# bark-simulator/planner-miqp

Measured on AMD Instinct MI355X. Metric: MIQP solves/sec to 1% gap, 2-agent x 20-step x 32-region, higher is better.
Workload: dtype f64

## Files before the change

### planner_miqp_amd/csrc/as_onchip.hip

```cpp
namespace miqp {

#ifdef MIQP_PROFILE
#define ASP_T(var) const long long var = clock64()
#define ASP_ACC(k, t0, t1) asp_[k] += (unsigned long long)((t1) - (t0))
#else
#define ASP_T(var)
#define ASP_ACC(k, t0, t1)
#endif
constexpr int AS_MAXSTEP = 220;
constexpr double AS_VTOL = 1.0e-8;
constexpr double AS_DEP = 1.0e-8;
constexpr int AS_MT = 64;
constexpr int AS_MSTR = AS_MT * (AS_MT + 1) / 2;

__host__ __device__ constexpr bool as_shape_ok(int C, int N) { return (C == 1 || C == 2) && N >= 1 && N <= 2 * OC_NSL; }

template <int C> __device__ inline int as_col(int pq) { return C == 2 ? ((pq & 3) << 2) | (pq >> 2) : ((pq & 1) << 2) | (pq >> 1); }
template <int C> __device__ inline int as_pcol(int q) { return C == 2 ? ((q & 3) << 2) | (q >> 2) : ((q & 3) << 1) | (q >> 2); }
template <int C> struct AsDecode {
  static constexpr bool LANE_BOUNDS = true, ROW_IDENTITY = true, MARKS = true;
  static __device__ int col(int l) { return as_col<C>(oc_pcol<C, true>(l)); }
};

template <int C, int NSL, int GCAP = miqp::OC_GCAP>
__global__ void __launch_bounds__(64, (GCAP > 128 ? 1 : 2)) as_onchip_kernel(DevBuf B) {
  static_assert(C == 1 || C == 2, "a stage of 16 columns holds the chains of up to two cars");
  constexpr bool CM = true;
  constexpr bool BIG = GCAP > 128;
  constexpr int OC_GCAP = GCAP, OC_GSLOTS = OC_GCAP / 64, OC_GCOEF = oc_gcoef_of(OC_GCAP);
  constexpr int NX = 6 * C, NZ = 8 * C, NCH = 2 * C;
  const Layout& Y = B.Y;
  const int tid = threadIdx.x, lg = tid >> 4, lc = tid & 15;
  const int par = lg >> 1, side = lg & 1;
  const double bsgn = side ? -1.0 : 1.0;
  WAVE_DUMP(BIG ? 1 : 4);
  const int* const clist = BIG && B.cls_take ? B.cls_list + (size_t)(B.cls_take - 1) * B.batch_cap : nullptr;
  const int nbatch = clist ? (B.cls_count[B.cls_take - 1] < B.batch_cap ? B.cls_count[B.cls_take - 1] : B.batch_cap) : (*B.batch_count < B.batch_cap ? *B.batch_count : B.batch_cap);
  const int N = Y.N, NSLOT = Y.NSLOT;
  extern __shared__ double lds[];
  char* const L0 = (char*)lds;
  const OcLds LL = oc_lds_layout(N, Y.fixlen, OC_GCAP, !BIG);
  double* const Z = (double*)(L0 + LL.z);
  double* const scr = (double*)(L0 + LL.u);
  double* const V = (double*)(L0 + LL.u);
  unsigned long long* const bkey = (unsigned long long*)(L0 + LL.r);
  const int SPAN = LL.gmeta - LL.u;
  double* const kref = (double*)(L0 + LL.u + SPAN - N * 32);
  double* const kff = kref - N * 4;
  double* const KS = kff - N * 16;
  const int STG_CAP = (SPAN - N * 192) / 8;
  uint4* const gmeta = (uint4*)(L0 + LL.gmeta);
  double* const gcoef = (double*)(L0 + LL.gcoef);
  double* const grhs = (double*)(L0 + LL.grhs);
  double* const Wd = (double*)(L0 + LL.wd);
  int* const sstart = (int*)(L0 + LL.sstart);
  unsigned short* const cand = (unsigned short*)(L0 + LL.cand);
  signed char* const fix = (signed char*)(L0 + LL.fix);
  __shared__ int sh_node;
  __shared__ unsigned long long sh_stat[32];
  if (tid < 32) sh_stat[tid] = 0ull;
  const unsigned long long lt = (1ull << tid) - 1ull;

  const int chunk = B.as_chunk > 0 ? B.as_chunk : 1;
  int run_next = 0, run_end = 0;
  const int quota = BIG ? 0 : B.as_quota; int handed = 0;
#ifdef MIQP_PROFILE
  const unsigned long long wv_c0 = __builtin_amdgcn_s_memtime(), wv_r0 = __builtin_amdgcn_s_memrealtime();
  unsigned long long wv_first = 0; int wv_nodes = 0;
  if (!BIG && tid == 0) wv_first = atomicMin(&B.prof[120], wv_r0);
#endif
  for (;;) {
    __syncthreads();
    if (run_next >= run_end) {
      if (quota > 0 && handed >= quota) break;
      ++handed;
      if (tid == 0) sh_node = atomicAdd(B.work_counter, chunk);
      __syncthreads();
      run_next = __builtin_amdgcn_readfirstlane(sh_node); run_end = run_next + chunk;
      if (run_next >= nbatch) break;
    }
    const int slot_ = run_next++;
    if (slot_ >= nbatch) { run_next = run_end; continue; }
    const int node = clist ? __builtin_amdgcn_readfirstlane(clist[slot_]) : slot_;
    {
      const int cls = B.batch_large ? (int)B.batch_large[node] : (is_probe_word(B.batch_depth[node]) ? 1 : 0);
      if (cls != (BIG ? 1 : 0)) continue;
    }
    WAVE_DUMP_NODE();
    const int inst = __builtin_amdgcn_readfirstlane(B.batch_inst[node]);
    const double* D = B.inst_d + (size_t)inst * Y.dstride;
    const int* T = B.inst_i + (size_t)inst * Y.istride;
    const double ts = D[Y.d_glob + 7];
    const double aqs = 2.0 * D[Y.d_misc + 0];
    const double iaq = aqs > 0.0 ? 1.0 / aqs : 0.0;
    {
      const signed char* src = B.pool_fix + (size_t)B.batch_node[node] * Y.fixlen;
      for (int k = tid; k < Y.fixlen; k += 64) fix[k] = src[k];
      if (tid < 16) Wd[tid] = tid < NZ ? D[Y.d_wd + oc_lcol<C, CM>(as_pcol<C>(tid))] : 0.0;
      for (int k = tid; k < N * 32; k += 64) bkey[k] = ~0ull;
      for (int k = tid; k <= N + 1; k += 64) sstart[k] = 0;
    }
    __syncthreads();
    const double* Rf = D + Y.d_ref;
    double cutoff = 1e300;
    {
      const double inc0 = fmin(inc_from_key(*(volatile unsigned long long*)&B.inc_key[inst]), B.inc_ext[inst]);
      const double gap_ = is_probe_word(B.batch_depth[node]) ? 0.0 : B.inst_gap[inst];
      if (B.use_cutoff && inc0 < 1e300) cutoff = inc0 - gap_ * (1e-10 + fabs(inc0)) - B.inst_const[inst];
    }

#ifdef MIQP_PROFILE
    unsigned long long asp_[12] = {0, 0, 0, 0, 0, 0, 0, 0, 0, 0, 0, 0};
#endif
    ASP_T(ta0);
#define OC_DECODE_POLICY AsDecode<C>
#include "oc_decode_body.inc"
#undef OC_DECODE_POLICY
    if (overflow) {
      if (B.batch_A) B.batch_A[(size_t)node * 64 + tid] = 0xFFFFu;
      if (tid == 0) {
        if (B.ring_M) B.batch_Mtag[node] = 0ull;
        B.batch_ok[node] = 5; B.pool_big[B.batch_node[node]] |= (BIG ? 2 : 1); if (B.stats) { atomicAdd(&B.stats[3], 1ull); atomicAdd(&B.stats[8 + (ngen >= 512 ? 15 : ngen / 32)], 1ull); }
      }
      continue;
    }
    const int NM = sstart[N + 1];
    OC_WAVE_SYNC();

    ASP_T(ta1); ASP_ACC(0, ta0, ta1);
#ifdef MIQP_PROFILE
    asp_[9] += (unsigned long long)(ocd_t_sparse - ta0); asp_[11] += (unsigned long long)(ta1 - ocd_t_rows);
#endif
    double brhs[NSL];
    unsigned int bact = 0u, binA = 0u, ginA = 0u;
#pragma unroll
    for (int k = 0; k < NSL; ++k) {
      const int i = 2 * k + par;
      brhs[k] = 1e300;
      if (i < N && lc < NZ) {
        const unsigned long long key = bkey[(i * 2 + side) * 16 + lc];
        if (key != ~0ull) { brhs[k] = key2d(key); bact |= 1u << k; }
      }
    }
    OC_WAVE_SYNC();

    const double h1 = ts, h2 = 0.5 * ts * ts, h3 = ts * ts * ts / 6.0;
    const double* const tb = D + Y.d_astab;
    if constexpr (C == 2) {
      for (int k = tid; k < N * 16; k += 64) KS[k] = tb[k];
      for (int k = tid; k < N * 4; k += 64) kref[k] = tb[N * 16 + k];
    } else {
      for (int k = tid; k < N * 8; k += 64) KS[(k >> 3) * 16 + (k & 7)] = tb[k];
      for (int k = tid; k < N * 2; k += 64) kref[(k >> 1) * 4 + (k & 1)] = tb[N * 8 + k];
    }
    OC_WAVE_SYNC();
    typedef double d2_t __attribute__((ext_vector_type(2)));
    auto subst = [&](const bool fromx0, const int itop, const int iend, double* const out) {
      for (int k = tid; k < (N - 1) * 4; k += 64) if ((k >> 2) > itop) kff[k] = fromx0 ? kref[k] : 0.0;
      if (tid < NCH) {
        const int ch = tid;
        double p0 = 0.0, p1 = 0.0, p2 = 0.0;
        int i0 = itop;
        if (itop >= N - 1) { const d2_t a = *(const d2_t*)(V + (N - 1) * 16 + 4 * ch); p0 = a[0]; p1 = a[1]; p2 = V[(N - 1) * 16 + 4 * ch + 2]; i0 = N - 2; }
        if (i0 >= 0) {
          d2_t va = *(const d2_t*)(V + i0 * 16 + 4 * ch), vb = *(const d2_t*)(V + i0 * 16 + 4 * ch + 2);
          d2_t ka = *(const d2_t*)(KS + (i0 * 4 + ch) * 4), kb = *(const d2_t*)(KS + (i0 * 4 + ch) * 4 + 2);
          double kr = fromx0 ? kref[i0 * 4 + ch] : 0.0;
          for (int i = i0; i >= 0; --i) {
            const int j = i > 0 ? i - 1 : 0;
            const d2_t nva = *(const d2_t*)(V + j * 16 + 4 * ch), nvb = *(const d2_t*)(V + j * 16 + 4 * ch + 2);
            const d2_t nka = *(const d2_t*)(KS + (j * 4 + ch) * 4), nkb = *(const d2_t*)(KS + (j * 4 + ch) * 4 + 2);
            const double nkr = fromx0 ? kref[j * 4 + ch] : 0.0;
            const double su = vb[1] + h3 * p0 + h2 * p1 + h1 * p2;
            const double sx0 = va[0] + p0, sx1 = va[1] + h1 * p0 + p1, sx2 = vb[0] + h2 * p0 + h1 * p1 + p2;
            kff[i * 4 + ch] = fma(su, kb[1], kr);
            p0 = sx0 - ka[0] * su; p1 = sx1 - ka[1] * su; p2 = sx2 - kb[0] * su;
            va = nva; vb = nvb; ka = nka; kb = nkb; kr = nkr;
          }
        }
      }
      OC_WAVE_SYNC();
      if (tid < NCH) {
        const int ch = tid;
        double x0 = 0.0, x1 = 0.0, x2 = 0.0;
        if (fromx0) { const int c = ch >> 1, s = ch & 1; x0 = D[Y.d_x0 + 6 * c + 3 * s]; x1 = D[Y.d_x0 + 6 * c + 3 * s + 1]; x2 = D[Y.d_x0 + 6 * c + 3 * s + 2]; }
        const int ie = iend < N - 1 ? iend : N - 2;
        d2_t ka = *(const d2_t*)(KS + ch * 4), kb = *(const d2_t*)(KS + ch * 4 + 2);
        double kf = kff[ch];
        for (int i = 0; i <= ie; ++i) {
          const int j = i < N - 2 ? i + 1 : N - 2;
          const d2_t nka = *(const d2_t*)(KS + (j * 4 + ch) * 4), nkb = *(const d2_t*)(KS + (j * 4 + ch) * 4 + 2);
          const double nkf = kff[j * 4 + ch];
          const double u = -kf - (ka[0] * x0 + ka[1] * x1 + kb[0] * x2);
          d2_t oa, ob; oa[0] = x0; oa[1] = x1; ob[0] = x2; ob[1] = u;
          *(d2_t*)(out + i * 16 + 4 * ch) = oa; *(d2_t*)(out + i * 16 + 4 * ch + 2) = ob;
          const double n0 = x0 + h1 * x1 + h2 * x2 + h3 * u, n1 = x1 + h1 * x2 + h2 * u, n2 = x2 + h1 * u;
// ... 438 lines not shown
```

### planner_miqp_amd/csrc/kernels.hip

```cpp
#include <hip/hip_runtime.h>

#include "host_inst.hpp"

#ifndef MIQP_RHO
#define MIQP_RHO 1.0e5
#endif

#ifndef MIQP_IPM_WPE
#define MIQP_IPM_WPE 3
#endif

#ifdef MIQP_ABLATE
#define MIQP_ABL (B.abl)
#else
#define MIQP_ABL 0
#endif
namespace miqp {

constexpr double RHO_EL = MIQP_RHO;
constexpr double FEAS_TOL = 1.0e-6;
constexpr double QP_TOL = 1.0e-6;
#ifndef MIQP_T0
#define MIQP_T0 1.0e-3
#endif
// ... 114 lines not shown
  double* ring_M; unsigned long long* ring_head; unsigned long long ring_doubles, ring_margin;
  unsigned long long* batch_Mtag;
  unsigned long long* pool_Mtag;
  int width_cap;
  int as_probe_first;
  int as_chunk;
  int* cls_list;
  int* cls_count;
  int cls_take;
  int lns_warm;
  int as_quota;
  int as_split;
  unsigned long long* as_stats;
};

__device__ inline unsigned long long d2key(double v) {
  unsigned long long u = (unsigned long long)__double_as_longlong(v);
  return (u & 0x8000000000000000ull) ? ~u : (u | 0x8000000000000000ull);
}
__device__ inline double key2d(unsigned long long k) {
  unsigned long long u = (k & 0x8000000000000000ull) ? (k & 0x7FFFFFFFFFFFFFFFull) : ~k;
  return __longlong_as_double((long long)u);
}

__device__ inline double inc_from_key(unsigned long long key) {
  if (key >= 0xFFF0000000000000ull) return 1e300;
  return key2d(key & ~0xFFFFFull);
}

template <int CTRL> __device__ inline double dpp_mov(double x) {
  int lo = __double2loint(x), hi = __double2hiint(x);
  lo = __builtin_amdgcn_update_dpp(lo, lo, CTRL, 0xF, 0xF, false);
  hi = __builtin_amdgcn_update_dpp(hi, hi, CTRL, 0xF, 0xF, false);
  return __hiloint2double(hi, lo);
}
__device__ inline void rows16(double x, double& even, double& odd) {
  const unsigned lo = (unsigned)__double2loint(x), hi = (unsigned)__double2hiint(x);
  const auto a = __builtin_amdgcn_permlane16_swap(lo, lo, false, false);
  const auto b = __builtin_amdgcn_permlane16_swap(hi, hi, false, false);
  even = __hiloint2double((int)b[0], (int)a[0]); odd = __hiloint2double((int)b[1], (int)a[1]);
}
__device__ inline void halves32(double x, double& lower, double& upper) {
  const unsigned lo = (unsigned)__double2loint(x), hi = (unsigned)__double2hiint(x);
  const auto a = __builtin_amdgcn_permlane32_swap(lo, lo, false, false);
  const auto b = __builtin_amdgcn_permlane32_swap(hi, hi, false, false);
  lower = __hiloint2double((int)b[0], (int)a[0]); upper = __hiloint2double((int)b[1], (int)a[1]);
}
__device__ inline double sum_xor16(double v) { double a, b; rows16(v, a, b); return a + b; }
__device__ inline double sum_xor32(double v) { double a, b; halves32(v, a, b); return a + b; }
__device__ inline double wave_min(double v) {
  v = fmin(v, dpp_mov<0xB1>(v)); v = fmin(v, dpp_mov<0x4E>(v)); v = fmin(v, dpp_mov<0x141>(v)); v = fmin(v, dpp_mov<0x140>(v));
  double a, b; rows16(v, a, b); v = fmin(a, b); halves32(v, a, b); return fmin(a, b);
}
__device__ inline double wave_max(double v) {
  v = fmax(v, dpp_mov<0xB1>(v)); v = fmax(v, dpp_mov<0x4E>(v)); v = fmax(v, dpp_mov<0x141>(v)); v = fmax(v, dpp_mov<0x140>(v));
  double a, b; rows16(v, a, b); v = fmax(a, b); halves32(v, a, b); return fmax(a, b);
}
__device__ inline double wave_sum(double v) {
  v += dpp_mov<0xB1>(v); v += dpp_mov<0x4E>(v); v += dpp_mov<0x141>(v); v += dpp_mov<0x140>(v);
  v = sum_xor16(v); return sum_xor32(v);
}

__device__ inline void add_point(double* g, double& rhs, int c, const double* rt, int tx, int ty, double al, double be, const double* K = nullptr) {
  g[6 * c + 0] += al;
  if (tx != PT_R) {
    if (rt) { const double* p = rt + 19 + (tx == PT_U ? 0 : 3); rhs -= al * p[0]; g[6 * c + 1] += al * p[1]; g[6 * c + 4] += al * p[2]; }
    else if (al != 0.0) rhs -= al * K[(tx == PT_U ? 0 : 2) + (al > 0.0 ? 0 : 1)];
  }
  g[6 * c + 3] += be;
  if (ty != PT_R) {
    if (rt) { const double* p = rt + 25 + (ty == PT_U ? 0 : 3); rhs -= be * p[0]; g[6 * c + 1] += be * p[1]; g[6 * c + 4] += be * p[2]; }
    else if (be != 0.0) rhs -= be * K[(ty == PT_U ? 4 : 6) + (be > 0.0 ? 0 : 1)];
  }
}


__device__ inline int env_corner(int tx, int ty) { return tx == PT_U ? (ty == PT_U ? 1 : 3) : (ty == PT_U ? 2 : 4); }
__device__ inline int obs_corner(int tx, int ty) { return tx == PT_L ? (ty == PT_L ? 1 : 3) : (ty == PT_L ? 2 : 4); }

__device__ inline bool corner_dominated(int tx, int ty, double al, double be, int domflag, int& txs, int& tys) {
  txs = al > 0.0 ? PT_U : (al < 0.0 ? PT_L : tx);
  tys = be > 0.0 ? PT_U : (be < 0.0 ? PT_L : ty);
  if (txs == tx && tys == ty) return false;
  if (txs != tx && !(domflag & 1)) return false;
  if (tys != ty && !(domflag & 2)) return false;
  return true;
}

__device__ inline void pair_cars(int p, int C, int& c1, int& c2) {
  c1 = 0; int rem = p;
  while (rem >= C - 1 - c1) { rem -= C - 1 - c1; ++c1; }
  c2 = c1 + 1 + rem;
}

struct RowOut { double rhs; double aq; bool active; };
__device__ inline int fix_stage(const Layout& Y, int k) {
  const int N = Y.N;
  if (k < Y.f_env) return (k - Y.f_reg) % N;
  if (k < Y.f_obs) return ((k - Y.f_env) / 5) % N;
  if (k < Y.f_c2c) return ((k - Y.f_obs) / 5) % N;
  if (k < Y.f_c2n) return ((k - Y.f_c2c) / 4) % N;
  return -1;
}
__device__ inline bool is_probe_word(int dw) { return (dw & 63) == 63 && (dw >> 6) >= 1; }
__device__ __forceinline__ double node_cutoff(const DevBuf& B, int inst, int node) {
  const double inc0 = fmin(inc_from_key(*(volatile unsigned long long*)&B.inc_key[inst]), B.inc_ext[inst]);
  if (!(B.use_cutoff && inc0 < 1e300)) return 1e300;
  return inc0 - (is_probe_word(B.batch_depth[node]) ? 0.0 : B.inst_gap[inst]) * (1e-10 + fabs(inc0)) - B.inst_const[inst];
}
#ifdef MIQP_PROFILE
struct WaveDump {
  const DevBuf& B; int kind; unsigned long long r0; int nodes;
  __device__ WaveDump(const DevBuf& b, int k) : B(b), kind(k), r0(__builtin_amdgcn_s_memrealtime()), nodes(0) {}
  __device__ ~WaveDump() {
    if (threadIdx.x == 0 && B.prof[125] == 300 && blockIdx.x < 4096) {
      unsigned int hw, xcc;
      asm volatile("s_getreg_b32 %0, hwreg(HW_REG_HW_ID)" : "=s"(hw));
      asm volatile("s_getreg_b32 %0, hwreg(HW_REG_XCC_ID)" : "=s"(xcc));
      unsigned long long* const w = B.prof + 160 + 4 * (kind * 4096 + blockIdx.x);
      w[0] = r0; w[1] = __builtin_amdgcn_s_memrealtime(); w[2] = ((unsigned long long)xcc << 32) | hw; w[3] = (unsigned long long)nodes;
    }
  }
};
#define WAVE_DUMP(kind) WaveDump wd_(B, kind)
#define WAVE_DUMP_NODE() (++wd_.nodes)
#else
#define WAVE_DUMP(kind)
#define WAVE_DUMP_NODE()
#endif
constexpr int CTR_SET = 16;
__device__ inline unsigned char large_class(const DevBuf& B, int rec, int dw, bool has_inc) {
  const unsigned int pb = B.pool_big ? (unsigned int)B.pool_big[rec] : 0u;
  const bool probe = is_probe_word(dw);
  if (!probe && !(pb & 0xF7u)) return 0;
  if (pb & 2u) return 3;
  if (pb & 4u) return 2;
  if (probe && B.pump_max > 0 && (!has_inc || B.pump_inc) && !B.as_probe_first) return 2;
  return 1;
}

__device__ inline int region_set(const Layout& Y, const int* T, const signed char* fix, int c, int i) {
  const int m = (int)(unsigned char)fix[Y.f_rmask + 2 * (c * Y.N + i)] | ((int)(unsigned char)fix[Y.f_rmask + 2 * (c * Y.N + i) + 1] << 8);
  return m & T[Y.i_rallow + c * Y.N + i];
}
__device__ inline const double* region_hull(const Layout& Y, const double* D, const int* T, const signed char* fix, int c, int i) {
  if (T[Y.i_nposs + c] > Y.PT) return D + Y.d_hull + (c * Y.N + i) * HULLSZ;
  return D + Y.d_hullm + (c * (1 << Y.PT) + region_set(Y, T, fix, c, i)) * 8;
}
__device__ inline const double* region_fpk(const Layout& Y, const double* D, const int* T, const signed char* fix, int c, int i) {
  if (T[Y.i_nposs + c] > Y.PT) return nullptr;
  return D + Y.d_fpk + (c * (1 << Y.PT) + region_set(Y, T, fix, c, i)) * 8;
}

template <int C, bool BUILD = true>
__device__ inline RowOut decode_row(const Layout& Y, const double* D, const int* T, const signed char* fix, int i, int slot, double* g) {
  constexpr int NZ = 8 * C;
  RowOut r; r.rhs = 0; r.aq = 0; r.active = false;
  if (BUILD) {
#pragma unroll
    for (int q = 0; q < NZ; ++q) g[q] = 0.0;
  }
  const int N = Y.N;
  const double* G = D + Y.d_glob;
  if (slot < C * Y.SC) {
    int c = slot / Y.SC, rr = slot - c * Y.SC;
    int code = i >= 1 ? (int)fix[Y.f_reg + c * N + i] : -1;
    const double* rt = code >= 0 ? D + Y.d_reg + (c * Y.P + (code >> 2)) * REGSZ : nullptr;
    const double* Hc = D + Y.d_hull + (c * N + i) * HULLSZ;
    if (rr < 7) {
      if (i < 1 || ((T[Y.i_boxskip + c * N + i] >> rr) & 1)) return r;
      r.active = true;
      if (!BUILD) return r;
      switch (rr) {
        case 0: g[6 * c + 1] = -1; r.rhs = -G[0]; break;
        case 1: g[6 * c + 4] = -1; r.rhs = -G[0]; break;
        case 2: g[6 * c + 1] = 1; r.rhs = G[1]; break;
        case 3: g[6 * c + 2] = 1; r.rhs = rt ? rt[12] : region_hull(Y, D, T, fix, c, i)[1]; break;
        case 4: g[6 * c + 2] = -1; r.rhs = -(rt ? rt[11] : region_hull(Y, D, T, fix, c, i)[0]); break;
        case 5: g[6 * c + 5] = 1; r.rhs = rt ? rt[14] : region_hull(Y, D, T, fix, c, i)[3]; break;
        default: g[6 * c + 5] = -1; r.rhs = -(rt ? rt[13] : region_hull(Y, D, T, fix, c, i)[2]); break;
      }
      return r;
    }
    if (rr < 11) {
      if (i > N - 2) return r;
      int s = (rr - 7) >> 1, up = ((rr - 7) & 1) == 0;
      double lo, hi;
      if (i == 0) { lo = D[Y.d_u0box + c * 4 + 2 * s]; hi = D[Y.d_u0box + c * 4 + 2 * s + 1]; }
      else if (rt) { lo = rt[15 + 2 * s]; hi = rt[16 + 2 * s]; }
      else if (!BUILD) { lo = hi = 0.0; }
      else { const double* Hm = region_hull(Y, D, T, fix, c, i); lo = Hm[4 + 2 * s]; hi = Hm[5 + 2 * s]; }
      r.active = true;
      if (!BUILD) return r;
      g[6 * C + 2 * c + s] = up ? 1.0 : -1.0; r.rhs = up ? hi : -lo;
      return r;
    }
    if (rr < 16) {
      if (i < 1) return r;
      if (code < 0) {
        const int k = rr - 11;
        if (k > 1 || Hc[14] == 0.0) return r;
        r.active = true; r.rhs = Hc[10 + 3 * k];
        if (!BUILD) return r;
        g[6 * c + 1] = Hc[8 + 3 * k]; g[6 * c + 4] = Hc[9 + 3 * k];
        return r;
      }
      int h = code & 3, k = rr - 11;
      if (h == 3) {
        if (k > 3) return r;
        r.active = true; r.rhs = G[6];
        if (!BUILD) return r;
        g[6 * c + (k < 2 ? 1 : 4)] = (k & 1) ? -1.0 : 1.0;
        return r;
      }
      r.active = true;
      if (!BUILD) return r;
      switch (k) {
        case 0: g[6 * c + 1] = rt[0]; g[6 * c + 4] = rt[1]; break;
        case 1: g[6 * c + 1] = rt[2]; g[6 * c + 4] = rt[3]; break;
        case 2: {
          const int* hs = T + Y.i_hs + ((c * Y.P + (code >> 2)) * 2 + h) * 2;
          g[6 * c + (hs[0] == 0 ? 1 : 4)] = -(double)hs[1]; r.rhs = -G[6];
        } break;
        case 3: g[6 * c + 5] = 1; g[6 * c + 2] = -rt[4]; g[6 * c + 1] = -rt[6]; g[6 * c + 4] = -rt[7]; r.rhs = rt[5]; break;
        default: g[6 * c + 5] = -1; g[6 * c + 2] = rt[4]; g[6 * c + 1] = rt[9]; g[6 * c + 4] = rt[10]; r.rhs = -rt[8]; break;
      }
      return r;
    }
    int q = rr - 16;
    if (q < 5 * Y.EL) {
      if (i < 1 || Y.E < 1) return r;
      int pt = q / Y.EL, k = q - pt * Y.EL;
      int e = Y.E == 1 ? 0 : (int)fix[Y.f_env + (c * N + i) * 5 + pt];
      if (e < 0 || k >= T[Y.i_envn + e] || (pt > 0 && code < 0)) return r;
      const double* ed = D + Y.d_env + (e * Y.EL + k) * 3;
      if (pt > 0) {
        int txs, tys;
        if (corner_dominated(ENV_PT_D[pt][0], ENV_PT_D[pt][1], ed[0], ed[1], T[Y.i_dom + (c * Y.P + (code >> 2)) * 4 + (code & 3)], txs, tys)) {
          int ps = env_corner(txs, tys);
          int es = Y.E == 1 ? 0 : (int)fix[Y.f_env + (c * N + i) * 5 + ps];
          if (es == e) return r;
        }
      }
      r.active = true; r.rhs = ed[2];
      if (!BUILD) return r;
      add_point(g, r.rhs, c, rt, ENV_PT_D[pt][0], ENV_PT_D[pt][1], ed[0], ed[1]);
      return r;
    }
    q -= 5 * Y.EL;
    int o = q / 5, pt = q - o * 5;
    if (i < 1) return r;
    int kk = (int)fix[Y.f_obs + ((c * Y.O + o) * N + i) * 5 + pt];
    if (kk < 0 || kk >= Y.L || (pt > 0 && code < 0)) return r;
    const double* ed = D + Y.d_obs + ((o * N + i) * Y.L + kk) * 3;
    if (pt > 0) {
      int txs, tys;
      if (corner_dominated(OBS_PT_D[pt][0], OBS_PT_D[pt][1], ed[0], ed[1], T[Y.i_dom + (c * Y.P + (code >> 2)) * 4 + (code & 3)], txs, tys)) {
        int ps = obs_corner(txs, tys);
        if ((int)fix[Y.f_obs + ((c * Y.O + o) * N + i) * 5 + ps] == kk) return r;
      }
    }
    r.active = true; r.rhs = ed[2];
    if (!BUILD) return r;
    add_point(g, r.rhs, c, rt, OBS_PT_D[pt][0], OBS_PT_D[pt][1], ed[0], ed[1]);
    return r;
  }
  if (C < 2 || i < 1) return r;
  int q = slot - C * Y.SC;
  const bool excl = q >= Y.NP * 8;
  int p, grp, which, alt;
  if (!excl) { p = q >> 3; grp = (q & 7) >> 1; which = q & 1; alt = (int)fix[Y.f_c2c + (p * N + i) * 4 + grp]; if (alt < 0) return r; }
  else {
    int q2 = q - Y.NP * 8; p = q2 >> 4; grp = (q2 >> 2) & 3; alt = q2 & 3; which = 1;
    int m = (int)fix[Y.f_c2n + (p * N + i) * 4 + grp];
    if (m <= 0 || !((m >> alt) & 1)) return r;
  }
  int c1, c2; pair_cars(p, C, c1, c2);
  int code1 = (int)fix[Y.f_reg + c1 * N + i], code2 = (int)fix[Y.f_reg + c2 * N + i];
  bool need1 = grp >= 2, need2 = (grp == 1 || grp == 3);
  const double* K1 = nullptr; const double* K2 = nullptr;
  if (need1 && code1 < 0) { if (excl || Y.relax_front_off) return r; K1 = region_fpk(Y, D, T, fix, c1, i); if (!K1) return r; }
  if (need2 && code2 < 0) { if (excl || Y.relax_front_off) return r; K2 = region_fpk(Y, D, T, fix, c2, i); if (!K2) return r; }
  const double* rt1 = code1 >= 0 ? D + Y.d_reg + (c1 * Y.P + (code1 >> 2)) * REGSZ : nullptr;
  const double* rt2 = code2 >= 0 ? D + Y.d_reg + (c2 * Y.P + (code2 >> 2)) * REGSZ : nullptr;
  double Dsep = D[Y.d_dsep + p * N + i], S = D[Y.d_ssl + i], smax = D[Y.d_smax + i], wsl = D[Y.d_misc + 0];
  bool soft = (grp == 0 || grp == 3);
  if (!excl) {
    if (!soft && which == 1) return r;
    if (soft && which == 1 && !(smax > 0 && wsl > 0)) return r;
  }
  bool isx = alt < 2, lo = (alt == 0 || alt == 2);
  int ca, cb, ta, tb;
  if (grp == 0) { ta = tb = PT_R; ca = lo ? c1 : c2; cb = lo ? c2 : c1; }
  else if (grp == 1) { if (lo) { ca = c1; ta = PT_R; cb = c2; tb = PT_L; } else { ca = c2; ta = PT_U; cb = c1; tb = PT_R; } }
  else if (grp == 2) { if (lo) { ca = c2; ta = PT_R; cb = c1; tb = PT_L; } else { ca = c1; ta = PT_U; cb = c2; tb = PT_R; } }
  else { if (lo) { ca = c2; ta = PT_U; cb = c1; tb = PT_L; } else { ca = c1; ta = PT_U; cb = c2; tb = PT_L; } }
  double al = isx ? 1.0 : 0.0, be = isx ? 0.0 : 1.0;
  r.active = true;
  if (!BUILD) return r;
  r.rhs = soft ? (which == 0 ? -(Dsep + S) + smax : -(Dsep + S)) : -Dsep;
  r.aq = (!excl && soft && which == 1) ? 2.0 * wsl : 0.0;
  add_point(g, r.rhs, ca, ca == c1 ? rt1 : rt2, ta, ta, al, be, ca == c1 ? K1 : K2);
  add_point(g, r.rhs, cb, cb == c1 ? rt1 : rt2, tb, tb, -al, -be, cb == c1 ? K1 : K2);
  if (excl) {
#pragma unroll
    for (int k = 0; k < NZ; ++k) g[k] = -g[k];
    r.rhs = -r.rhs;
  }
  return r;
}

template <int C>
__device__ inline double ab_entry(int q, int b, double ts) {
  constexpr int NX = 6 * C;
  int ch = q / 3, k = q - 3 * ch;
  if (b < NX) {
    int chb = b / 3, kb = b - 3 * chb;
    if (chb != ch || kb < k) return 0.0;
    int d = kb - k;
    return d == 0 ? 1.0 : (d == 1 ? ts : 0.5 * ts * ts);
  }
  if (b - NX != ch) return 0.0;
  return k == 0 ? ts * ts * ts / 6.0 : (k == 1 ? 0.5 * ts * ts : ts);
}

struct RowRegs { double aq, col, s, lam, t, v[6]; };
__device__ inline RowRegs load_row(const double* rc_aq, const double* rc_col, const double* rc_v, const double* rs_s, const double* rs_l,
                                   const double* rs_t, int rowcap, int idx) {
  RowRegs R;
  R.aq = rc_aq[idx]; R.col = rc_col[idx]; R.s = rs_s[idx]; R.lam = rs_l[idx]; R.t = rs_t[idx];
#pragma unroll
  for (int k = 0; k < 6; ++k) R.v[k] = rc_v[(size_t)k * rowcap + idx];
  return R;
}

__device__ inline void lds_barrier() { asm volatile("s_waitcnt lgkmcnt(0)\n\ts_barrier" ::: "memory"); }

template <int NT> __device__ inline double block_sum(double v, double* red) {
  v = wave_sum(v);
  if constexpr (NT > 64) { __syncthreads(); if ((threadIdx.x & 63) == 0) red[threadIdx.x >> 6] = v; __syncthreads(); v = 0.0;
#pragma unroll
    for (int w = 0; w < NT / 64; ++w) v += red[w]; }
  return v;
}
template <int NT> __device__ inline double block_min(double v, double* red) {
  v = wave_min(v);
  if constexpr (NT > 64) { __syncthreads(); if ((threadIdx.x & 63) == 0) red[threadIdx.x >> 6] = v; __syncthreads(); v = red[0];
#pragma unroll
    for (int w = 1; w < NT / 64; ++w) v = fmin(v, red[w]); }
  return v;
}
template <int NT> __device__ inline double block_max(double v, double* red) {
  v = wave_max(v);
  if constexpr (NT > 64) { __syncthreads(); if ((threadIdx.x & 63) == 0) red[threadIdx.x >> 6] = v; __syncthreads(); v = red[0];
#pragma unroll
    for (int w = 1; w < NT / 64; ++w) v = fmax(v, red[w]); }
  return v;
}

#ifdef MIQP_PROFILE
#define PROF_T(var) long long var = clock64()
#define PROF_ACC(k, t0, t1) pr_[k] += (unsigned long long)((t1) - (t0))
#else
#define PROF_T(var)
#define PROF_ACC(k, t0, t1)
#endif

__device__ inline double readlane_d(double v, int lane) {
  int lo = __builtin_amdgcn_readlane(__double2loint(v), lane), hi = __builtin_amdgcn_readlane(__double2hiint(v), lane);
  return __hiloint2double(hi, lo);
}

__device__ inline double frcp(double x) {
  double r = __builtin_amdgcn_rcp(x);
  return fma(r, fma(-x, r, 1.0), r);
}
__device__ inline double frsq(double x) {
  double r = __builtin_amdgcn_rsq(x);
  return fma(0.5 * r, fma(-x * r, r, 1.0), r);
}

__device__ inline void init_elastic(double c, bool warm, double mu0, double delta, double& s, double& lam, double& t) {
  if (!warm) {
    if (c > QP_T0) { t = QP_T0; s = c + QP_T0; } else { s = MIQP_S0 * QP_T0; t = s - c; }
    lam = MIQP_LAM0;
    return;
  }
  s = c > delta ? c : delta;
  lam = mu0 / s; if (lam > 0.5 * RHO_EL) lam = 0.5 * RHO_EL;
  double tt = mu0 / (RHO_EL - lam);
  if (s - c > tt) tt = s - c;
  t = tt; s = c + tt;
}

__device__ inline void row_step(double s, double lam, double t, double aq, double gd, double tau, double& ds, double& dl, double& dt) {
  const double il = frcp(lam);
  const double r1 = tau - s * lam;
  double zz, r2m = 0.0, im = 0.0, r2 = 0.0;
  if (aq == 0.0) { const double mu = RHO_EL - lam; im = frcp(mu); zz = t * im; r2 = tau - t * mu; r2m = r2 * im; }
  else zz = frcp(aq);
  const double w = frcp(s * il + zz);
  dl = (gd + r1 * il - r2m) * w;
  ds = (r1 - s * dl) * il;
  dt = aq == 0.0 ? (r2 + t * dl) * im : 0.0;
}

#ifndef MIQP_WIDE_WPE
#define MIQP_WIDE_WPE 2
#endif
#ifndef MIQP_WIDE_NT
#define MIQP_WIDE_NT 128
#endif
template <int C, int NT>
__global__ void __launch_bounds__(NT, (C <= 2 ? MIQP_IPM_WPE : (NT > 64 ? MIQP_WIDE_WPE : 1))) ipm_kernel(DevBuf B) {
  static_assert(C <= 4, "stage vectors of at most 32 entries");
  constexpr bool WIDE = C > 2;
  static_assert(NT == 64 || (WIDE && (NT == 128 || NT == 256)), "one wavefront per node, or two / four for the 2 x 2-tiled stage algebra");
  constexpr int NW = NT / 64;
  constexpr int NX = 6 * C, NU = 2 * C, NZ = 8 * C, GS = WIDE ? NZ + 1 : GSTR;
  constexpr int KB = (NX + 3) / 4;
  constexpr int RU = NX / 4, GU0 = NX % 4;
  const Layout& Y = B.Y;
  const int tid = threadIdx.x;
  WAVE_DUMP(3);
  const int* const clist = B.cls_take ? B.cls_list + (size_t)(B.cls_take - 1) * B.batch_cap : nullptr;
  const int nbatch = clist ? (B.cls_count[B.cls_take - 1] < B.batch_cap ? B.cls_count[B.cls_take - 1] : B.batch_cap) : B.ovf_mode == 1 ? *B.ovf_count : (*B.batch_count < B.batch_cap ? *B.batch_count : B.batch_cap);
  const int N = Y.N, NSLOT = Y.NSLOT;
  extern __shared__ double lds[];
  double* Z = lds;
  double* dZ = Z + N * NZ;
  double* Gh = dZ + N * NZ;
  double* fs = Gh + GROWS * GS;
  double* Wd = Z + N * NZ + ipm_scratch_doubles(N, C);
  double* red = Wd + NZ;
  double* dgq = red + 8;
  int* sstart = (int*)(dgq + 32);
  int* sst = sstart + ((N + 4) & ~1);
  signed char* fix = (signed char*)(sst + ((N + 4) & ~1));
  double* dscr = dZ;
  constexpr int KSTR = NX + 2;
// ... 2238 lines not shown
```

### planner_miqp_amd/csrc/oc_decode_body.inc

```
#ifdef MIQP_PROFILE
    long long ocd_t_sparse = 0, ocd_t_rows = 0;
#endif
    int ngen = 0;
    {
      unsigned long long* const bmp = (unsigned long long*)scr;
      const int nw = (N * NSLOT + 63) >> 6;
      unsigned short* const pre = (unsigned short*)(bmp + nw);
      for (int k = tid; k < nw; k += 64) bmp[k] = 0ull;
      OC_WAVE_SYNC();
      const int cls_off[8] = {0, 7, 11, 16, 16 + Y.EL, 16 + 5 * Y.EL, C * Y.SC, C * Y.SC + 8 * Y.NP};
      const int cls_cnt[8] = {7, 4, 5, Y.EL, 4 * Y.EL, 5 * Y.O, 8 * Y.NP, 16 * Y.NP};
      auto take = [&](int i, int slot) {
        if (decode_row<C, false>(Y, D, T, fix, i, slot, nullptr).active) {
          int col; double sg, rh;
          if (box_of_slot<C>(Y, D, T, fix, i, slot, col, sg, rh)) atomicMin(&bkey[(i * 2 + (sg < 0.0 ? 1 : 0)) * 16 + OC_DECODE_POLICY::col(col)], d2key(rh));
          else { const int pcode = i * NSLOT + slot; atomicOr(&bmp[pcode >> 6], 1ull << (pcode & 63)); }
        }
      };
      unsigned short* const plist = pre + ((nw + 1 + 3) & ~3);
      const int LCAP = (int)(((char*)(L0 + LL.r) - (char*)plist) / 2) - 64;
      int nlist = 0;
      auto flush = [&]() {
        OC_WAVE_SYNC();
        for (int j0 = 0; j0 < nlist; j0 += 64) if (j0 + tid < nlist) { const int pc = plist[j0 + tid]; const int i = pc / NSLOT; take(i, pc - i * NSLOT); }
        OC_WAVE_SYNC();
        nlist = 0;
      };
      if constexpr (OC_DECODE_POLICY::LANE_BOUNDS) {
        for (int e0 = 0; e0 < C * N; e0 += 64) {
          const int e = e0 + tid;
          if (e < C * N) {
            const int c = e / N, i = e - c * N;
            const double* G = D + Y.d_glob;
            const int code = i >= 1 ? (int)fix[Y.f_reg + c * N + i] : -1;
            const unsigned int skip = i >= 1 ? (unsigned int)T[Y.i_boxskip + c * N + i] : 0x7Fu;
            const double* rt = code >= 0 ? D + Y.d_reg + (c * Y.P + (code >> 2)) * REGSZ : nullptr;
            const double* Hc = (!rt && i >= 1) ? region_hull(Y, D, T, fix, c, i) : nullptr;
            auto put = [&](int col, bool neg, double rh) { atomicMin(&bkey[(i * 2 + (neg ? 1 : 0)) * 16 + OC_DECODE_POLICY::col(col)], d2key(rh)); };
            if (i >= 1) {
              const double a_lo_x = rt ? rt[11] : Hc[0], a_hi_x = rt ? rt[12] : Hc[1], a_lo_y = rt ? rt[13] : Hc[2], a_hi_y = rt ? rt[14] : Hc[3];
              if (!(skip & 1u)) put(6 * c + 1, true, -G[0]);
              if (!(skip & 2u)) put(6 * c + 4, true, -G[0]);
              if (!(skip & 4u)) put(6 * c + 1, false, G[1]);
              if (!(skip & 8u)) put(6 * c + 2, false, a_hi_x);
              if (!(skip & 16u)) put(6 * c + 2, true, -a_lo_x);
              if (!(skip & 32u)) put(6 * c + 5, false, a_hi_y);
              if (!(skip & 64u)) put(6 * c + 5, true, -a_lo_y);
            }
            if (i <= N - 2) {
#pragma unroll
              for (int s_ = 0; s_ < 2; ++s_) {
                double lo, hi;
                if (i == 0) { lo = D[Y.d_u0box + c * 4 + 2 * s_]; hi = D[Y.d_u0box + c * 4 + 2 * s_ + 1]; }
                else if (rt) { lo = rt[15 + 2 * s_]; hi = rt[16 + 2 * s_]; }
                else { lo = Hc[4 + 2 * s_]; hi = Hc[5 + 2 * s_]; }
                put(6 * C + 2 * c + s_, false, hi); put(6 * C + 2 * c + s_, true, -lo);
              }
            }
          }
        }
      }
#pragma unroll 1
      for (int cl = 0; cl < 8; ++cl) {
#ifdef MIQP_PROFILE
        if (OC_DECODE_POLICY::MARKS && cl == 2) ocd_t_sparse = clock64();
#endif
        const int cnt = cls_cnt[cl], off = cls_off[cl];
        const bool percar = cl < 6;
        const int per = percar ? C * cnt : cnt, total = N * per;
        for (int e0 = 0; e0 < total; e0 += 64) {
          const int e = e0 + tid;
          int i = 0, slot = 0; bool in = e < total;
          if (in) { i = e / per; const int rem = e - i * per; slot = percar ? (rem / cnt) * Y.SC + off + rem % cnt : off + rem; }
          if (cl < 2) {
            if constexpr (!OC_DECODE_POLICY::LANE_BOUNDS) { if (in) take(i, slot); }
            continue;
          }
          const bool cnd = in && slot_maybe<C>(Y, fix, i, slot);
          const unsigned long long mk = __ballot(cnd);
          if (cnd) plist[nlist + __popcll(mk & lt)] = (unsigned short)(i * NSLOT + slot);
          nlist += __popcll(mk);
          if (nlist > LCAP) flush();
        }
      }
      flush();
      if (tid == 0) { int a = 0; for (int k = 0; k < nw; ++k) { pre[k] = (unsigned short)(a < 65535 ? a : 65535); a += __popcll(bmp[k]); } pre[nw] = (unsigned short)(a < 65535 ? a : 65535); }
      OC_WAVE_SYNC();
      ngen = pre[nw];
      if (ngen <= OC_GCAP)
        for (int k = tid; k < nw; k += 64) {
          unsigned long long bits = bmp[k]; int pos = pre[k];
          while (bits) { const int b = __ffsll((long long)bits) - 1; cand[pos++] = (unsigned short)(k * 64 + b); bits &= bits - 1ull; }
        }
      OC_WAVE_SYNC();
    }
#ifdef MIQP_PROFILE
    if (OC_DECODE_POLICY::MARKS) ocd_t_rows = clock64();
#endif
    bool overflow = ngen > OC_GCAP;
    int ncoef = 0;
    for (int c0 = 0; c0 < ngen && !overflow; c0 += OC_SCR) {
      double* g = scr + (tid & (OC_SCR - 1)) * OC_SSTR;
      RowOut r; r.active = false; r.rhs = 0; r.aq = 0;
      int i = 0, nn = 0;
      const bool mine = tid < OC_SCR && c0 + tid < ngen;
      int slot_ = 0;
      if (mine) { const int pcode = cand[c0 + tid]; i = pcode / NSLOT; slot_ = pcode - i * NSLOT; r = decode_row<C, true>(Y, D, T, fix, i, slot_, g); }
      unsigned long long map = 0ull; unsigned int cols = 0u;
      double v6[6];
#pragma unroll
      for (int k = 0; k < 6; ++k) v6[k] = 0.0;
      if (mine) {
        for (int q = 0; q < NZ; ++q) {
          const double v = g[q];
          if (v != 0.0 && nn < 6) {
#pragma unroll
            for (int k = 0; k < 6; ++k) if (k == nn) v6[k] = v;
            const int pq = OC_DECODE_POLICY::col(q);
            map |= (unsigned long long)(nn + 1) << (4 * pq); cols |= (unsigned int)pq << (4 * nn); nn++;
          }
        }
      }
      const bool keep = mine && nn > 0;
      const unsigned long long mk = __ballot(keep);
      const unsigned long long b0 = __ballot(keep && (nn & 1)), b1 = __ballot(keep && (nn & 2)), b2 = __ballot(keep && (nn & 4));
      const int tot = __popcll(b0) + 2 * __popcll(b1) + 4 * __popcll(b2);
      if (ncoef + tot > OC_GCOEF) { overflow = true; break; }
      if (keep) {
        const int idx = sstart[N + 1] + __popcll(mk & lt);
        const int off = ncoef + __popcll(b0 & lt) + 2 * __popcll(b1 & lt) + 4 * __popcll(b2 & lt);
#pragma unroll
        for (int k = 0; k < 6; ++k) if (k < nn) gcoef[off + k] = v6[k];
        uint4 m4; m4.x = (unsigned int)map; m4.y = (unsigned int)(map >> 32);
        m4.z = (unsigned int)off | ((unsigned int)nn << 16) | ((unsigned int)i << 20) | (r.aq > 0.0 ? 0x80000000u : 0u); m4.w = cols;
        gmeta[idx] = m4; grhs[idx] = r.rhs;
        if constexpr (OC_DECODE_POLICY::ROW_IDENTITY) cand[idx] = (unsigned short)(i * NSLOT + slot_);
        else atomicAdd(&sstart[i + 1], 1);
      }
      OC_WAVE_SYNC();
      if (tid == 0) sstart[N + 1] += __popcll(mk);
      ncoef += tot;
      OC_WAVE_SYNC();
    }
```

Measured before the change: 1088.

## Decode candidate rows class-sorted across full wave with skipped re-checks and compaction pass

Row decoding now sorts candidates by constraint class, so neighbouring lanes take the same branch in decode_row. It uses all 64 lanes with a larger scratch area that now starts at the Z region instead of OC_SCR lanes. A TESTED template flag skips validity checks already done by the earlier slot_maybe filter. Rows are written at their original rank, then compacted back into candidate order in a second register-staged pass. This trades extra compaction work and more LDS scratch for less divergence and more decode parallelism. It relies on the candidate filter matching the skipped checks exactly and on scratch not overlapping live data.

```diff
diff --git a/planner_miqp_amd/csrc/as_onchip.hip b/planner_miqp_amd/csrc/as_onchip.hip
--- a/planner_miqp_amd/csrc/as_onchip.hip
+++ b/planner_miqp_amd/csrc/as_onchip.hip
@@ -41,7 +41,7 @@
   char* const L0 = (char*)lds;
   const OcLds LL = oc_lds_layout(N, Y.fixlen, OC_GCAP, !BIG);
   double* const Z = (double*)(L0 + LL.z);
-  double* const scr = (double*)(L0 + LL.u);
+  double* const scr = (double*)(L0 + LL.z);
   double* const V = (double*)(L0 + LL.u);
   unsigned long long* const bkey = (unsigned long long*)(L0 + LL.r);
   const int SPAN = LL.gmeta - LL.u;
diff --git a/planner_miqp_amd/csrc/kernels.hip b/planner_miqp_amd/csrc/kernels.hip
--- a/planner_miqp_amd/csrc/kernels.hip
+++ b/planner_miqp_amd/csrc/kernels.hip
@@ -290,7 +290,7 @@
   return D + Y.d_fpk + (c * (1 << Y.PT) + region_set(Y, T, fix, c, i)) * 8;
 }
 
-template <int C, bool BUILD = true>
+template <int C, bool BUILD = true, bool TESTED = false>
 __device__ inline RowOut decode_row(const Layout& Y, const double* D, const int* T, const signed char* fix, int i, int slot, double* g) {
   constexpr int NZ = 8 * C;
   RowOut r; r.rhs = 0; r.aq = 0; r.active = false;
@@ -337,7 +337,7 @@
       if (i < 1) return r;
       if (code < 0) {
         const int k = rr - 11;
-        if (k > 1 || Hc[14] == 0.0) return r;
+        if (!TESTED && (k > 1 || Hc[14] == 0.0)) return r;
         r.active = true; r.rhs = Hc[10 + 3 * k];
         if (!BUILD) return r;
         g[6 * c + 1] = Hc[8 + 3 * k]; g[6 * c + 4] = Hc[9 + 3 * k];
@@ -370,9 +370,9 @@
       if (i < 1 || Y.E < 1) return r;
       int pt = q / Y.EL, k = q - pt * Y.EL;
       int e = Y.E == 1 ? 0 : (int)fix[Y.f_env + (c * N + i) * 5 + pt];
-      if (e < 0 || k >= T[Y.i_envn + e] || (pt > 0 && code < 0)) return r;
+      if (!TESTED && (e < 0 || k >= T[Y.i_envn + e] || (pt > 0 && code < 0))) return r;
       const double* ed = D + Y.d_env + (e * Y.EL + k) * 3;
-      if (pt > 0) {
+      if (!TESTED && pt > 0) {
         int txs, tys;
         if (corner_dominated(ENV_PT_D[pt][0], ENV_PT_D[pt][1], ed[0], ed[1], T[Y.i_dom + (c * Y.P + (code >> 2)) * 4 + (code & 3)], txs, tys)) {
           int ps = env_corner(txs, tys);
@@ -389,9 +389,9 @@
     int o = q / 5, pt = q - o * 5;
     if (i < 1) return r;
     int kk = (int)fix[Y.f_obs + ((c * Y.O + o) * N + i) * 5 + pt];
-    if (kk < 0 || kk >= Y.L || (pt > 0 && code < 0)) return r;
+    if (!TESTED && (kk < 0 || kk >= Y.L || (pt > 0 && code < 0))) return r;
     const double* ed = D + Y.d_obs + ((o * N + i) * Y.L + kk) * 3;
-    if (pt > 0) {
+    if (!TESTED && pt > 0) {
       int txs, tys;
       if (corner_dominated(OBS_PT_D[pt][0], OBS_PT_D[pt][1], ed[0], ed[1], T[Y.i_dom + (c * Y.P + (code >> 2)) * 4 + (code & 3)], txs, tys)) {
         int ps = obs_corner(txs, tys);
@@ -423,7 +423,7 @@
   const double* rt2 = code2 >= 0 ? D + Y.d_reg + (c2 * Y.P + (code2 >> 2)) * REGSZ : nullptr;
   double Dsep = D[Y.d_dsep + p * N + i], S = D[Y.d_ssl + i], smax = D[Y.d_smax + i], wsl = D[Y.d_misc + 0];
   bool soft = (grp == 0 || grp == 3);
-  if (!excl) {
+  if (!TESTED && !excl) {
     if (!soft && which == 1) return r;
     if (soft && which == 1 && !(smax > 0 && wsl > 0)) return r;
   }
diff --git a/planner_miqp_amd/csrc/oc_decode_body.inc b/planner_miqp_amd/csrc/oc_decode_body.inc
--- a/planner_miqp_amd/csrc/oc_decode_body.inc
+++ b/planner_miqp_amd/csrc/oc_decode_body.inc
@@ -99,46 +99,106 @@
 #endif
     bool overflow = ngen > OC_GCAP;
     int ncoef = 0;
-    for (int c0 = 0; c0 < ngen && !overflow; c0 += OC_SCR) {
-      double* g = scr + (tid & (OC_SCR - 1)) * OC_SSTR;
-      RowOut r; r.active = false; r.rhs = 0; r.aq = 0;
-      int i = 0, nn = 0;
-      const bool mine = tid < OC_SCR && c0 + tid < ngen;
-      int slot_ = 0;
-      if (mine) { const int pcode = cand[c0 + tid]; i = pcode / NSLOT; slot_ = pcode - i * NSLOT; r = decode_row<C, true>(Y, D, T, fix, i, slot_, g); }
-      unsigned long long map = 0ull; unsigned int cols = 0u;
-      double v6[6];
-#pragma unroll
-      for (int k = 0; k < 6; ++k) v6[k] = 0.0;
-      if (mine) {
-        for (int q = 0; q < NZ; ++q) {
-          const double v = g[q];
-          if (v != 0.0 && nn < 6) {
-#pragma unroll
-            for (int k = 0; k < 6; ++k) if (k == nn) v6[k] = v;
-            const int pq = OC_DECODE_POLICY::col(q);
-            map |= (unsigned long long)(nn + 1) << (4 * pq); cols |= (unsigned int)pq << (4 * nn); nn++;
-          }
-        }
-      }
-      const bool keep = mine && nn > 0;
-      const unsigned long long mk = __ballot(keep);
-      const unsigned long long b0 = __ballot(keep && (nn & 1)), b1 = __ballot(keep && (nn & 2)), b2 = __ballot(keep && (nn & 4));
-      const int tot = __popcll(b0) + 2 * __popcll(b1) + 4 * __popcll(b2);
-      if (ncoef + tot > OC_GCOEF) { overflow = true; break; }
-      if (keep) {
-        const int idx = sstart[N + 1] + __popcll(mk & lt);
-        const int off = ncoef + __popcll(b0 & lt) + 2 * __popcll(b1 & lt) + 4 * __popcll(b2 & lt);
-#pragma unroll
-        for (int k = 0; k < 6; ++k) if (k < nn) gcoef[off + k] = v6[k];
-        uint4 m4; m4.x = (unsigned int)map; m4.y = (unsigned int)(map >> 32);
-        m4.z = (unsigned int)off | ((unsigned int)nn << 16) | ((unsigned int)i << 20) | (r.aq > 0.0 ? 0x80000000u : 0u); m4.w = cols;
-        gmeta[idx] = m4; grhs[idx] = r.rhs;
-        if constexpr (OC_DECODE_POLICY::ROW_IDENTITY) cand[idx] = (unsigned short)(i * NSLOT + slot_);
-        else atomicAdd(&sstart[i + 1], 1);
-      }
-      OC_WAVE_SYNC();
-      if (tid == 0) sstart[N + 1] += __popcll(mk);
-      ncoef += tot;
-      OC_WAVE_SYNC();
+    if (!overflow) {
+      constexpr int OC_RPL = OC_GCAP / 64;
+      unsigned short* const ord = (unsigned short*)((char*)(L0 + LL.r) - 2 * OC_GCAP);
+      const int nfit = (int)(((char*)ord - (char*)scr) / (OC_SSTR * 8)), nrow = nfit < 64 ? nfit : 64;
+      {
+        const int ncar = C * Y.SC;
+        unsigned int clp = 0u;
+#pragma unroll
+        for (int q = 0; q < OC_RPL; ++q) {
+          const int k = tid + 64 * q;
+          if (k < ngen) {
+            const int pc = cand[k], slot = pc - (pc / NSLOT) * NSLOT, rr = slot % Y.SC;
+            const int cl = slot >= ncar ? (slot < ncar + 8 * Y.NP ? 6 : 7) : (rr < 16 ? 2 : (rr < 16 + Y.EL ? 3 : (rr < 16 + 5 * Y.EL ? 4 : 5)));
+            clp |= (unsigned int)cl << (4 * q);
+          }
+        }
+        int base = 0;
+#pragma unroll 1
+        for (int cl = 2; cl < 8; ++cl) {
+#pragma unroll
+          for (int q = 0; q < OC_RPL; ++q) {
+            const bool is = (int)((clp >> (4 * q)) & 15u) == cl;
+            const unsigned long long mk = __ballot(is);
+            if (is) ord[base + __popcll(mk & lt)] = (unsigned short)(tid + 64 * q);
+            base += __popcll(mk);
+          }
+        }
+      }
+      OC_WAVE_SYNC();
+      for (int c0 = 0; c0 < ngen; c0 += nrow) {
+        double* g = scr + tid * OC_SSTR;
+        RowOut r; r.active = false; r.rhs = 0; r.aq = 0;
+        int i = 0, nn = 0, rank = 0;
+        const bool mine = tid < nrow && c0 + tid < ngen;
+        if (mine) { rank = ord[c0 + tid]; const int pcode = cand[rank]; i = pcode / NSLOT; r = decode_row<C, true, true>(Y, D, T, fix, i, pcode - i * NSLOT, g); }
+        unsigned long long map = 0ull; unsigned int cols = 0u;
+        double v6[6];
+#pragma unroll
+        for (int k = 0; k < 6; ++k) v6[k] = 0.0;
+        if (mine) {
+          for (int q = 0; q < NZ; ++q) {
+            const double v = g[q];
+            if (v != 0.0 && nn < 6) {
+#pragma unroll
+              for (int k = 0; k < 6; ++k) if (k == nn) v6[k] = v;
+              const int pq = OC_DECODE_POLICY::col(q);
+              map |= (unsigned long long)(nn + 1) << (4 * pq); cols |= (unsigned int)pq << (4 * nn); nn++;
+            }
+          }
+        }
+        const unsigned long long b0 = __ballot(nn & 1), b1 = __ballot(nn & 2), b2 = __ballot(nn & 4);
+        const int tot = __popcll(b0) + 2 * __popcll(b1) + 4 * __popcll(b2);
+        if (ncoef + tot > OC_GCOEF) { overflow = true; break; }
+        if (mine) {
+          const int off = ncoef + __popcll(b0 & lt) + 2 * __popcll(b1 & lt) + 4 * __popcll(b2 & lt);
+#pragma unroll
+          for (int k = 0; k < 6; ++k) if (k < nn) gcoef[off + k] = v6[k];
+          uint4 m4; m4.x = (unsigned int)map; m4.y = (unsigned int)(map >> 32);
+          m4.z = (unsigned int)off | ((unsigned int)nn << 16) | ((unsigned int)i << 20) | (r.aq > 0.0 ? 0x80000000u : 0u); m4.w = cols;
+          gmeta[rank] = m4; grhs[rank] = r.rhs;
+        }
+        ncoef += tot;
+      }
+      OC_WAVE_SYNC();
+      if (!overflow) {
+        uint4 pm[OC_RPL]; double prh[OC_RPL], pv[OC_RPL][6]; int ppc[OC_RPL];
+#pragma unroll
+        for (int q = 0; q < OC_RPL; ++q) {
+          const int k = tid + 64 * q;
+          pm[q] = make_uint4(0u, 0u, 0u, 0u); prh[q] = 0.0; ppc[q] = 0;
+#pragma unroll
+          for (int j = 0; j < 6; ++j) pv[q][j] = 0.0;
+          if (k < ngen) {
+            pm[q] = gmeta[k]; prh[q] = grhs[k]; ppc[q] = cand[k];
+            const int off = (int)(pm[q].z & 0xFFFFu), nn = (int)((pm[q].z >> 16) & 15u);
+#pragma unroll
+            for (int j = 0; j < 6; ++j) if (j < nn) pv[q][j] = gcoef[off + j];
+          }
+        }
+        OC_WAVE_SYNC();
+        int nkept = 0, co = 0;
+#pragma unroll
+        for (int q = 0; q < OC_RPL; ++q) {
+          const int nn = (int)((pm[q].z >> 16) & 15u);
+          const bool keep = nn > 0;
+          const unsigned long long mk = __ballot(keep);
+          const unsigned long long b0 = __ballot(nn & 1), b1 = __ballot(nn & 2), b2 = __ballot(nn & 4);
+          if (keep) {
+            const int idx = nkept + __popcll(mk & lt);
+            const int off = co + __popcll(b0 & lt) + 2 * __popcll(b1 & lt) + 4 * __popcll(b2 & lt);
+#pragma unroll
+            for (int j = 0; j < 6; ++j) if (j < nn) gcoef[off + j] = pv[q][j];
+            uint4 m4 = pm[q]; m4.z = (m4.z & 0xFFFF0000u) | (unsigned int)off;
+            gmeta[idx] = m4; grhs[idx] = prh[q];
+            if constexpr (OC_DECODE_POLICY::ROW_IDENTITY) cand[idx] = (unsigned short)ppc[q];
+            else atomicAdd(&sstart[((m4.z >> 20) & 0x7FFu) + 1], 1);
+          }
+          nkept += __popcll(mk); co += __popcll(b0) + 2 * __popcll(b1) + 4 * __popcll(b2);
+        }
+        if (tid == 0) sstart[N + 1] = nkept;
+        OC_WAVE_SYNC();
+      }
     }
```

New measurement: 1086. About the same (-0.2%).
